# Human-Augment-Analytics/vectordb-retrieval

Hardware: AMD Instinct MI355X
Metric: QPS @ recall@10 (SIFT1M-shaped, 10k-query batch, k=10) (higher is better)
Workload: dtype i8 MFMA scan (i32 accumulate) + exact integer / f64 refine

## Files before the change

### vectordb-retrieval_amd/csrc/refine.hpp

```cpp
#pragma once
#include "common.hpp"
#include "topk.hpp"

namespace vdb {

struct Sq8Rows {
    const unsigned char *codes = nullptr;
    const int32_t *list = nullptr;
    const float *cent = nullptr;
    const float *vmin = nullptr;
    const float *vdiff = nullptr;
};

__device__ __forceinline__ float sq8_decode(unsigned code, float c, float vmin, float vdiff) {
    return c + (vmin + (((float)code + 0.5f) / 255.0f) * vdiff);
}

struct PqRows {
    const unsigned char *codes = nullptr;
    const float *cb = nullptr;
    int M = 0, dsub = 0;
};

struct IvfPqRows {
    const int32_t *list = nullptr;
    const float *cent = nullptr;
    PqRows pq{};
};

struct RefineCommon {
    const float *X;
    const float *Q;
    int64_t N;
    int64_t id_base;
    int D4;
    int metric;
    int k;
    const int64_t *idmap;
    const signed char *X8 = nullptr;
    const int *rowstat = nullptr;
    const signed char *Q8 = nullptr;
    int x8_pitch = 0, cx = 0, D = 0;
    const QueryBatchInfo *info = nullptr;
    Sq8Rows sq8{};
    PqRows pq{};
    IvfPqRows ivfpq{};
};

typedef int refine_int4 __attribute__((ext_vector_type(4)));

template <int U = 16>
__device__ __forceinline__ uint64_t exact_key(const float *__restrict__ x, const float *__restrict__ q, int D4,
                                              int metric) {
    const float4 *xv = reinterpret_cast<const float4 *>(x);
    const float4 *qv = reinterpret_cast<const float4 *>(q);
    double acc = 0.0;
    if (metric == 0) {
#pragma unroll U
        for (int i = 0; i < D4 / 4; ++i) {
            const float4 a = xv[i];
            const float4 b = qv[i];
            double t;
            t = (double)a.x - (double)b.x; acc = fma(t, t, acc);
            t = (double)a.y - (double)b.y; acc = fma(t, t, acc);
            t = (double)a.z - (double)b.z; acc = fma(t, t, acc);
            t = (double)a.w - (double)b.w; acc = fma(t, t, acc);
        }
        return sortable_u64(acc);
    } else {
#pragma unroll U
        for (int i = 0; i < D4 / 4; ++i) {
            const float4 a = xv[i];
            const float4 b = qv[i];
            acc = fma((double)b.x, (double)a.x, acc);
            acc = fma((double)b.y, (double)a.y, acc);
            acc = fma((double)b.z, (double)a.z, acc);
            acc = fma((double)b.w, (double)a.w, acc);
        }
        return sortable_u64(-acc);
    }
}

template <int U = 16>
__device__ __forceinline__ uint64_t exact_key_i8(const signed char *__restrict__ x8, int cx, const float *__restrict__ q,
                                                 int D4, int metric) {
    const int *xw = reinterpret_cast<const int *>(x8);
    const float4 *qv = reinterpret_cast<const float4 *>(q);
    double acc = 0.0;
#pragma unroll U
    for (int i = 0; i < D4 / 4; ++i) {
        const int w = xw[i];
        const float4 b = qv[i];
        const double x0 = (double)((int)(signed char)(w & 0xff) + cx), x1 = (double)((int)(signed char)((w >> 8) & 0xff) + cx);
        const double x2 = (double)((int)(signed char)((w >> 16) & 0xff) + cx), x3 = (double)((w >> 24) + cx);
        if (metric == 0) {
            double t;
            t = x0 - (double)b.x; acc = fma(t, t, acc);
            t = x1 - (double)b.y; acc = fma(t, t, acc);
            t = x2 - (double)b.z; acc = fma(t, t, acc);
            t = x3 - (double)b.w; acc = fma(t, t, acc);
        } else {
            acc = fma((double)b.x, x0, acc);
            acc = fma((double)b.y, x1, acc);
            acc = fma((double)b.z, x2, acc);
            acc = fma((double)b.w, x3, acc);
        }
    }
    return sortable_u64(metric == 0 ? acc : -acc);
}

__device__ __forceinline__ uint64_t sq8_key(const Sq8Rows &s, int64_t row, const float *__restrict__ q, int D4, int metric) {
    const unsigned *cw = reinterpret_cast<const unsigned *>(s.codes + (size_t)row * D4);
    const float4 *cv = reinterpret_cast<const float4 *>(s.cent + (size_t)s.list[row] * D4);
    const float4 *mv = reinterpret_cast<const float4 *>(s.vmin);
    const float4 *dv = reinterpret_cast<const float4 *>(s.vdiff);
    const float4 *qv = reinterpret_cast<const float4 *>(q);
    double acc = 0.0;
#pragma unroll 4
    for (int i = 0; i < D4 / 4; ++i) {
        const unsigned w = cw[i];
        const float4 c = cv[i], m = mv[i], d = dv[i], b = qv[i];
        const double x0 = (double)sq8_decode(w & 0xffu, c.x, m.x, d.x);
        const double x1 = (double)sq8_decode((w >> 8) & 0xffu, c.y, m.y, d.y);
        const double x2 = (double)sq8_decode((w >> 16) & 0xffu, c.z, m.z, d.z);
        const double x3 = (double)sq8_decode(w >> 24, c.w, m.w, d.w);
        if (metric == 0) {
            double t;
            t = x0 - (double)b.x; acc = fma(t, t, acc);
            t = x1 - (double)b.y; acc = fma(t, t, acc);
            t = x2 - (double)b.z; acc = fma(t, t, acc);
            t = x3 - (double)b.w; acc = fma(t, t, acc);
        } else {
            acc = fma((double)b.x, x0, acc);
            acc = fma((double)b.y, x1, acc);
            acc = fma((double)b.z, x2, acc);
            acc = fma((double)b.w, x3, acc);
        }
    }
    return sortable_u64(metric == 0 ? acc : -acc);
}

template <bool RESIDUAL>
__device__ __forceinline__ uint64_t pq_key_body(const PqRows &p, const int32_t *__restrict__ list, const float *__restrict__ cent,
                                                int64_t row, const float *__restrict__ q, int D4, int metric) {
    const unsigned char *cr = p.codes + (size_t)row * p.M;
    const float *cl = RESIDUAL ? cent + (size_t)list[row] * D4 : nullptr;
    double acc = 0.0;
    int d = 0;
    for (int m = 0; m < p.M; ++m) {
        const float *cv = p.cb + ((size_t)m * 256 + cr[m]) * p.dsub;
        for (int j = 0; j < p.dsub; ++j, ++d) {
            const double x = RESIDUAL ? (double)(cl[d] + cv[j]) : (double)cv[j];
            if (metric == 0) {
                const double t = x - (double)q[d];
                acc = fma(t, t, acc);
            } else {
                acc = fma((double)q[d], x, acc);
            }
        }
    }
    for (; d < D4; ++d) {
        if (metric == 0) {
            const double t = 0.0 - (double)q[d];
            acc = fma(t, t, acc);
        } else {
            acc = fma((double)q[d], 0.0, acc);
        }
    }
    return sortable_u64(metric == 0 ? acc : -acc);
}
__device__ __forceinline__ uint64_t pq_key(const PqRows &p, int64_t row, const float *__restrict__ q, int D4, int metric) {
    return pq_key_body<false>(p, nullptr, nullptr, row, q, D4, metric);
}
__device__ __forceinline__ uint64_t ivfpq_key(const IvfPqRows &p, int64_t row, const float *__restrict__ q, int D4, int metric) {
    return pq_key_body<true>(p.pq, p.list, p.cent, row, q, D4, metric);
}

template <int U = 16>
__device__ __forceinline__ uint64_t row_key(const RefineCommon &c, int64_t row, const float *__restrict__ q) {
    if (c.X) return exact_key<U>(c.X + (size_t)row * c.D4, q, c.D4, c.metric);
    if (c.sq8.codes) return sq8_key(c.sq8, row, q, c.D4, c.metric);
    if (c.pq.codes) return pq_key(c.pq, row, q, c.D4, c.metric);
    if (c.ivfpq.pq.codes) return ivfpq_key(c.ivfpq, row, q, c.D4, c.metric);
    return exact_key_i8<U>(c.X8 + (size_t)row * c.x8_pitch, c.cx, q, c.D4, c.metric);
}

template <int QB>
__device__ __forceinline__ void exact_keys(const float *__restrict__ x, const float *const (&q)[QB], int D4, int metric,
                                           uint64_t (&out)[QB]) {
    const float4 *xv = reinterpret_cast<const float4 *>(x);
    double acc[QB];
#pragma unroll
    for (int j = 0; j < QB; ++j) acc[j] = 0.0;
#pragma unroll 4
    for (int i = 0; i < D4 / 4; ++i) {
        const float4 a = xv[i];
#pragma unroll
        for (int j = 0; j < QB; ++j) {
            const float4 b = reinterpret_cast<const float4 *>(q[j])[i];
            if (metric == 0) {
                double t;
                t = (double)a.x - (double)b.x; acc[j] = fma(t, t, acc[j]);
                t = (double)a.y - (double)b.y; acc[j] = fma(t, t, acc[j]);
                t = (double)a.z - (double)b.z; acc[j] = fma(t, t, acc[j]);
                t = (double)a.w - (double)b.w; acc[j] = fma(t, t, acc[j]);
            } else {
                acc[j] = fma((double)b.x, (double)a.x, acc[j]);
                acc[j] = fma((double)b.y, (double)a.y, acc[j]);
                acc[j] = fma((double)b.z, (double)a.z, acc[j]);
                acc[j] = fma((double)b.w, (double)a.w, acc[j]);
            }
        }
    }
#pragma unroll
    for (int j = 0; j < QB; ++j) out[j] = sortable_u64(metric == 0 ? acc[j] : -acc[j]);
}

template <int KPL, int U = 16>
__device__ __forceinline__ void scan_rows(WaveTopK<KPL> &tk, const RefineCommon &c, const float *qptr, int64_t row0,
                                          int64_t row1) {
    const int lane = threadIdx.x & 63;
    if (row1 > c.N) row1 = c.N;
    for (int64_t base = row0; base < row1; base += 64) {
        const int64_t row = base + lane;
        const bool valid = row < row1;
        uint64_t key = ~0ull;
        if (valid) key = row_key<U>(c, row, qptr);
        tk.offer(key, c.idmap ? (valid ? c.idmap[row] : -1) : c.id_base + row, valid);
    }
}

template <int KPL>
__device__ __forceinline__ void write_topk(const WaveTopK<KPL> &tk, int metric, float *D, int64_t *I, double *pk,
                                           int64_t *pi) {
    const int lane = threadIdx.x & 63;
#pragma unroll
    for (int e = 0; e < KPL; ++e) {
        const int s = e * 64 + lane;
        if (s < tk.k) {
            const bool have = s < tk.n;
            const double kv = have ? unsortable_f64(tk.key[e]) : __builtin_inf();
            if (D) {
                float d;
                if (have)
                    d = (float)(metric == 0 ? kv : -kv);
                else
                    d = (metric == 0) ? 3.402823466e+38f : -3.402823466e+38f;
                D[s] = d;
                I[s] = have ? tk.id[e] : -1;
            } else {
                pk[s] = kv;
                pi[s] = have ? tk.id[e] : -1;
            }
        }
    }
}

struct RefineListArgs {
    RefineCommon c;
    int64_t nq;
    const int32_t *cand_rows;
    const int32_t *rescan_rows;
    const int32_t *counts;
    const int32_t *fallback;
    int cand_cap;
    int rescan_cap;
    float *D;
    int64_t *I;
    double *pkeys;
    int64_t *pids;
    int group_shift = -1;
    int f16_shift = 2;
};

template <int KPL, int W>
__device__ __forceinline__ void refine_list_dot8(const RefineListArgs &a, int64_t q, int ncand, int nres, int gshift,
                                                 WaveTopK<KPL> &tk) {
    const int lane = threadIdx.x & 63;
    const RefineCommon &c = a.c;
    const int mode = c.info->i8_mode;
    const int cq = (mode & 3) == 1 ? 127 : -1;
    int qb[W];
    const int *q8 = reinterpret_cast<const int *>(c.Q8 + (size_t)q * c.x8_pitch);
#pragma unroll
    for (int w = 0; w < W; ++w) qb[w] = __builtin_amdgcn_readfirstlane(q8[w]);
    int sq = 0, sqq = 0;
    const float *qf = c.Q + (size_t)q * c.D4;
    for (int d = lane; d < c.D4; d += 64) {
        const int v = (int)qf[d];
        sq += v;
        sqq += v * v;
    }
#pragma unroll
    for (int o = 32; o > 0; o >>= 1) {
        sq += __shfl_xor(sq, o);
        sqq += __shfl_xor(sqq, o);
    }
    const long long cxq = (long long)c.cx * sq - (long long)c.D * c.cx * cq;
    auto key_of = [&](int64_t row) -> uint64_t {
        const refine_int4 *xr = reinterpret_cast<const refine_int4 *>(c.X8 + (size_t)row * c.x8_pitch);
        const int2 st = reinterpret_cast<const int2 *>(c.rowstat)[row];
        int dot = 0;
#pragma unroll
        for (int i = 0; i < W / 4; ++i) {
            const refine_int4 w = xr[i];
            dot = __builtin_amdgcn_sdot4(w.x, qb[4 * i], dot, false);
            dot = __builtin_amdgcn_sdot4(w.y, qb[4 * i + 1], dot, false);
            dot = __builtin_amdgcn_sdot4(w.z, qb[4 * i + 2], dot, false);
            dot = __builtin_amdgcn_sdot4(w.w, qb[4 * i + 3], dot, false);
        }
        const long long xq = -(long long)dot + (long long)cq * st.y + cxq;
        return c.metric == 0 ? sortable_u64((double)((long long)st.x - 2 * xq + sqq)) : sortable_u64(-(double)xq);
    };
    const int32_t *cr = a.cand_rows + (size_t)q * a.cand_cap;
    for (int base = 0; base < (ncand << gshift); base += 64) {
        const int i = base + lane;
        bool valid = i < (ncand << gshift);
        const int64_t row = valid ? (int64_t)cr[i >> gshift] + (i & ((1 << gshift) - 1)) : 0;
        valid = valid && row < c.N;
        const uint64_t key = valid ? key_of(row) : ~0ull;
        tk.offer(key, c.idmap ? (valid ? c.idmap[row] : -1) : c.id_base + row, valid);
    }
    const int32_t *rr = a.rescan_rows + (size_t)q * a.rescan_cap * 2;
    for (int r = 0; r < nres; ++r) {
        const int64_t row0 = rr[2 * r];
        int64_t row1 = rr[2 * r + 1];
        if (row1 > c.N) row1 = c.N;
        for (int64_t base = row0; base < row1; base += 64) {
            const int64_t row = base + lane;
            const bool valid = row < row1;
            const uint64_t key = valid ? key_of(row) : ~0ull;
            tk.offer(key, c.idmap ? (valid ? c.idmap[row] : -1) : c.id_base + row, valid);
        }
    }
}

template <int KPL>
__device__ __forceinline__ void refine_list_body(const RefineListArgs &a, unsigned block) {
    const int lane = threadIdx.x & 63;
    const int64_t q = __builtin_amdgcn_readfirstlane((int)(block * 4 + (threadIdx.x >> 6)));
    if (q >= a.nq) return;
    if (a.fallback[q]) return;
    const float *qptr = a.c.Q + (size_t)q * a.c.D4;
    WaveTopK<KPL> tk;
    tk.init(a.c.k);
    int ncand = a.counts[2 * q];
    int nres = a.counts[2 * q + 1];
    ncand = ncand < a.cand_cap ? ncand : a.cand_cap;
    nres = nres < a.rescan_cap ? nres : a.rescan_cap;
    const int32_t *cr = a.cand_rows + (size_t)q * a.cand_cap;
    const int mode = a.c.info != nullptr ? a.c.info->i8_mode : 0;
    const int gshift = a.group_shift >= 0 ? a.group_shift : mode ? ((mode & 4) ? 3 : 2) : a.f16_shift;
    if (mode != 0 && a.c.X8 != nullptr) {
        if (a.c.x8_pitch == 64) refine_list_dot8<KPL, 16>(a, q, ncand, nres, gshift, tk);
        else refine_list_dot8<KPL, 32>(a, q, ncand, nres, gshift, tk);
    } else {
        for (int base = 0; base < (ncand << gshift); base += 64) {
            const int i = base + lane;
            bool valid = i < (ncand << gshift);
            int64_t row = valid ? (int64_t)cr[i >> gshift] + (i & ((1 << gshift) - 1)) : 0;
            valid = valid && row < a.c.N;
            uint64_t key = ~0ull;
            if (valid) key = row_key(a.c, row, qptr);
            tk.offer(key, a.c.idmap ? (valid ? a.c.idmap[row] : -1) : a.c.id_base + row, valid);
        }
        const int32_t *rr = a.rescan_rows + (size_t)q * a.rescan_cap * 2;
        for (int r = 0; r < nres; ++r) scan_rows<KPL>(tk, a.c, qptr, rr[2 * r], rr[2 * r + 1]);
    }
    const size_t o = (size_t)q * a.c.k;
    write_topk<KPL>(tk, a.c.metric, a.D ? a.D + o : nullptr, a.I ? a.I + o : nullptr, a.pkeys ? a.pkeys + o : nullptr,
                    a.pids ? a.pids + o : nullptr);
}

struct RefineFallbackArgs {
    RefineCommon c;
    const int32_t *fb_list;
    const int32_t *fb_count;
    int max_split;
    int64_t cap_units;
    double *pkeys;
    int64_t *pids;
    int32_t *done;
    float *D;
    int64_t *I;
    double *okeys;
    int64_t *oids;
};

template <int KPL>
__device__ __forceinline__ void refine_fallback_body(const RefineFallbackArgs &a, unsigned block, unsigned nblocks) {
    const int64_t count = *a.fb_count;
    if (count <= 0) return;
    const int lane = threadIdx.x & 63;
    const int64_t waves = (int64_t)nblocks * 4;
    const int64_t wave0 = __builtin_amdgcn_readfirstlane((int)(block * 4 + (threadIdx.x >> 6)));
    int64_t S = waves / count;
    if (S > a.max_split) S = a.max_split;
    if (S > a.cap_units / count) S = a.cap_units / count;
    if (S < 1) S = 1;
    const int64_t rows_per_split = ((a.c.N + S - 1) / S + 63) / 64 * 64;
    for (int64_t u = wave0; u < count * S; u += waves) {
        const int64_t f = u / S;
        const int split = (int)(u - f * S);
        const int64_t q = a.fb_list[f];
        WaveTopK<KPL> tk;
        tk.init(a.c.k);
        scan_rows<KPL, 4>(tk, a.c, a.c.Q + (size_t)q * a.c.D4, (int64_t)split * rows_per_split, (int64_t)(split + 1) * rows_per_split);
        const size_t oq = (size_t)q * a.c.k;
        if (S == 1) {
            if (a.D) write_topk<KPL>(tk, a.c.metric, a.D + oq, a.I + oq, nullptr, nullptr);
            else write_topk<KPL>(tk, a.c.metric, nullptr, nullptr, a.okeys + oq, a.oids + oq);
            continue;
        }
        write_topk<KPL>(tk, a.c.metric, nullptr, nullptr, a.pkeys + (size_t)u * a.c.k, a.pids + (size_t)u * a.c.k);
        __threadfence();
        int last = 0;
        if (lane == 0) last = atomicAdd(&a.done[f], 1) == (int)S - 1;
        last = __builtin_amdgcn_readfirstlane(last);
        if (!last) continue;
        __threadfence();
        if (lane == 0) a.done[f] = 0;
        tk.init(a.c.k);
        const int total = (int)S * a.c.k;
        const size_t o0 = (size_t)f * S * a.c.k;
        for (int base = 0; base < total; base += 64) {
            const int i = base + lane;
            bool valid = i < total;
            uint64_t key = ~0ull;
            int64_t id = -1;
            if (valid) {
                id = __builtin_nontemporal_load(a.pids + o0 + i);
                key = sortable_u64(__builtin_nontemporal_load(a.pkeys + o0 + i));
                valid = id >= 0;
            }
            tk.offer(key, id, valid);
        }
        if (a.D) write_topk<KPL>(tk, a.c.metric, a.D + oq, a.I + oq, nullptr, nullptr);
        else write_topk<KPL>(tk, a.c.metric, nullptr, nullptr, a.okeys + oq, a.oids + oq);
    }
}

template <int KPL>
__global__ __launch_bounds__(256, (KPL == 1 ? 6 : KPL == 2 ? 5 : 1)) void refine_tail_kernel(RefineListArgs la, RefineFallbackArgs fa, unsigned fb_blocks) {
    if (blockIdx.x < fb_blocks) refine_fallback_body<KPL>(fa, blockIdx.x, fb_blocks);
    else refine_list_body<KPL>(la, blockIdx.x - fb_blocks);
}

struct RerankArgs {
    RefineCommon c;
    int64_t nq;
    const int64_t *cand;
    int ncand;
    float *D;
    int64_t *I;
    double *pkeys = nullptr;
    int64_t *pids = nullptr;
    const int64_t *segs = nullptr;
    int nseg = 0;
};

template <int KPL>
__global__ __launch_bounds__(256) void rerank_kernel(RerankArgs a) {
    const int lane = threadIdx.x & 63;
    const int64_t q = __builtin_amdgcn_readfirstlane((int)(blockIdx.x * 4 + (threadIdx.x >> 6)));
    if (q >= a.nq) return;
    const float *qptr = a.c.Q + (size_t)q * a.c.D4;
    WaveTopK<KPL> tk;
    tk.init(a.c.k);
    const int64_t *cr = a.cand + (size_t)q * a.ncand;
    for (int base = 0; base < a.ncand; base += 64) {
        const int i = base + lane;
        bool valid = i < a.ncand;
        const int64_t id = valid ? cr[i] : -1;
        int64_t row = id - a.c.id_base;
        if (a.segs) {
            row = -1;
            for (int j = 0; j < a.nseg; ++j) {
                const int64_t id0 = a.segs[3 * j];
                if (id >= id0 && id < id0 + a.segs[3 * j + 2]) row = a.segs[3 * j + 1] + (id - id0);
            }
        }
        valid = valid && id >= 0 && row >= 0 && row < a.c.N;
        uint64_t key = ~0ull;
        if (valid) key = row_key(a.c, row, qptr);
        tk.offer(key, id, valid);
    }
    const size_t o = (size_t)q * a.c.k;
    write_topk<KPL>(tk, a.c.metric, a.D ? a.D + o : nullptr, a.I ? a.I + o : nullptr, a.pkeys ? a.pkeys + o : nullptr,
                    a.pids ? a.pids + o : nullptr);
}

struct RefineFullArgs {
    RefineCommon c;
    const int32_t *qlist;
    const int32_t *count_ptr;
    int64_t count;
    int S;
    int64_t rows_per_split;
    float *D;
    int64_t *I;
    double *pkeys;
    int64_t *pids;
};

template <int KPL>
__global__ __launch_bounds__(256) void refine_full_kernel(RefineFullArgs a) {
    const int64_t waves_total = (int64_t)gridDim.x * 4;
    const int64_t wave0 = __builtin_amdgcn_readfirstlane((int)(blockIdx.x * 4 + (threadIdx.x >> 6)));
    const int64_t count = a.count_ptr ? (int64_t)*a.count_ptr : a.count;
    const int64_t units = count * a.S;
    for (int64_t u = wave0; u < units; u += waves_total) {
        const int64_t slot = u / a.S;
        const int split = (int)(u - slot * a.S);
        const int64_t q = a.qlist ? (int64_t)a.qlist[slot] : slot;
        const float *qptr = a.c.Q + (size_t)q * a.c.D4;
        WaveTopK<KPL> tk;
        tk.init(a.c.k);
        const int64_t r0 = (int64_t)split * a.rows_per_split;
        scan_rows<KPL>(tk, a.c, qptr, r0, r0 + a.rows_per_split);
        if (a.D) {
            const size_t o = (size_t)q * a.c.k;
            write_topk<KPL>(tk, a.c.metric, a.D + o, a.I + o, nullptr, nullptr);
        } else {
            const size_t o = (size_t)u * a.c.k;
            write_topk<KPL>(tk, a.c.metric, nullptr, nullptr, a.pkeys + o, a.pids + o);
        }
    }
}

template <int KPL, int QB, bool PQ = false>
__global__ __launch_bounds__(256) void refine_full_blocked_kernel(RefineFullArgs a) {
    const int lane = threadIdx.x & 63;
    const int64_t waves_total = (int64_t)gridDim.x * 4;
    const int64_t wave0 = __builtin_amdgcn_readfirstlane((int)(blockIdx.x * 4 + (threadIdx.x >> 6)));
    const int64_t count = a.count_ptr ? (int64_t)*a.count_ptr : a.count;
    const int64_t groups = (count + QB - 1) / QB;
    const int64_t units = groups * a.S;
    for (int64_t u = wave0; u < units; u += waves_total) {
        const int64_t grp = u / a.S;
        const int split = (int)(u - grp * a.S);
        int64_t slot[QB], q[QB];
        const float *qptr[QB];
        WaveTopK<KPL> tk[QB];
#pragma unroll
        for (int j = 0; j < QB; ++j) {
            slot[j] = grp * QB + j;
            const int64_t sj = slot[j] < count ? slot[j] : count - 1;
            q[j] = a.qlist ? (int64_t)a.qlist[sj] : sj;
            qptr[j] = a.c.Q + (size_t)q[j] * a.c.D4;
            tk[j].init(a.c.k);
        }
        const int64_t r0 = (int64_t)split * a.rows_per_split;
        int64_t r1 = r0 + a.rows_per_split;
        if (r1 > a.c.N) r1 = a.c.N;
        for (int64_t base = r0; base < r1; base += 64) {
            const int64_t row = base + lane;
            const bool valid = row < r1;
            uint64_t key[QB];
#pragma unroll
            for (int j = 0; j < QB; ++j) key[j] = ~0ull;
            if (valid) {
                if (PQ) {
#pragma unroll
                    for (int j = 0; j < QB; ++j) key[j] = pq_key(a.c.pq, row, qptr[j], a.c.D4, a.c.metric);
                } else if (a.c.X) {
                    exact_keys<QB>(a.c.X + (size_t)row * a.c.D4, qptr, a.c.D4, a.c.metric, key);
                } else {
#pragma unroll
                    for (int j = 0; j < QB; ++j)
                        key[j] = exact_key_i8<4>(a.c.X8 + (size_t)row * a.c.x8_pitch, a.c.cx, qptr[j], a.c.D4, a.c.metric);
                }
            }
            const int64_t id = a.c.idmap ? (valid ? a.c.idmap[row] : -1) : a.c.id_base + row;
#pragma unroll
            for (int j = 0; j < QB; ++j) tk[j].offer(key[j], id, valid);
        }
#pragma unroll
        for (int j = 0; j < QB; ++j) {
            if (slot[j] < count) {
                if (a.D) {
                    const size_t o = (size_t)q[j] * a.c.k;
                    write_topk<KPL>(tk[j], a.c.metric, a.D + o, a.I + o, nullptr, nullptr);
                } else {
                    const size_t o = (size_t)(slot[j] * a.S + split) * a.c.k;
                    write_topk<KPL>(tk[j], a.c.metric, nullptr, nullptr, a.pkeys + o, a.pids + o);
                }
            }
        }
    }
}

struct MergeArgs {
    const double *pkeys;
    const int64_t *pids;
    int64_t part_stride;
    int64_t slot_stride;
    int nparts;
    int k;
    int metric;
    const int32_t *qlist;
    const int32_t *count_ptr;
    int64_t count;
    float *D;
    int64_t *I;
    double *okeys;
    int64_t *oids;
    const int64_t *seg;
};

template <int KPL>
__global__ __launch_bounds__(256) void merge_kernel(MergeArgs a) {
    const int lane = threadIdx.x & 63;
    const int64_t waves_total = (int64_t)gridDim.x * 4;
    const int64_t wave0 = __builtin_amdgcn_readfirstlane((int)(blockIdx.x * 4 + (threadIdx.x >> 6)));
    const int64_t count = a.count_ptr ? (int64_t)*a.count_ptr : a.count;
    const int total = a.nparts * a.k;
    for (int64_t slot = wave0; slot < count; slot += waves_total) {
        WaveTopK<KPL> tk;
        tk.init(a.k);
        for (int base = 0; base < total; base += 64) {
            const int i = base + lane;
            bool valid = i < total;
            uint64_t key = ~0ull;
            int64_t id = -1;
            if (valid) {
                const int p = i / a.k, j = i - p * a.k;
                const size_t o = (size_t)p * a.part_stride + (size_t)slot * a.slot_stride + j;
                id = a.pids[o];
                key = sortable_u64(a.pkeys[o]);
                valid = id >= 0;
                if (valid && a.seg) {
                    const int64_t *pairs = a.seg + a.nparts + 1;
                    int64_t e = a.seg[p];
                    const int64_t e1 = a.seg[p + 1];
                    while (e + 1 < e1 && pairs[2 * (e + 1)] <= id) ++e;
                    id = pairs[2 * e + 1] + (id - pairs[2 * e]);
                }
            }
            tk.offer(key, id, valid);
        }
        const int64_t q = a.qlist ? (int64_t)a.qlist[slot] : slot;
        const size_t o = (size_t)q * a.k;
        if (a.D)
            write_topk<KPL>(tk, a.metric, a.D + o, a.I + o, nullptr, nullptr);
        else
            write_topk<KPL>(tk, a.metric, nullptr, nullptr, a.okeys + o, a.oids + o);
    }
}

}
```

### vectordb-retrieval_amd/csrc/scan.hpp

```cpp
#pragma once
#include "common.hpp"
#include "prep.hpp"

namespace vdb {

typedef float float16v __attribute__((ext_vector_type(16)));

struct ScanArgs {
    const half8 *panels;
    const float *bias;
    const half8 *qpanels;
    const QueryBatchInfo *info;
    float *bin_m1;
    float *bin_m2;
    float *bin_m3;
    float *sb_m1;
    float *sb_m2;
    int32_t *sb_span;
    int64_t nspans;
    int spans_per_chunk;
    int chunk_rem;
    int nchunks;
    int chunk0;
    int nqtiles;
// ... 235 lines not shown
            }
        }
    };
    auto flush_bin = [&](int64_t span, int bt) {
        if (ITEMS) {
            items_push((int)(span - lspan0) * BPS + bt);
            return;
        }
        const size_t o = (size_t)((span * 2 + h) * BPS + bt) * out_pitch + out_col;
#pragma unroll
        for (int cb = 0; cb < 2; ++cb) {
            __builtin_nontemporal_store(m1[cb], a.bin_m1 + o + cb * 32);
            __builtin_nontemporal_store(m2[cb], a.bin_m2 + o + cb * 32);
            M2[cb] = __builtin_fminf(__builtin_amdgcn_fmed3f(M1[cb], M2[cb], m1[cb]), m2[cb]);
            if (m1[cb] < M1[cb]) Ms[cb] = (int)span;
            M1[cb] = __builtin_fminf(M1[cb], m1[cb]);
            m1[cb] = INF;
            m2[cb] = INF;
        }
    };

    stage_issue(0, 0);
    if (ITEMS) {
        const half8 *ra = reinterpret_cast<const half8 *>(a.qrows + (size_t)(qa < 0 ? 0 : qa) * (16 * KSTEPS)) + h;
        const half8 *rb = reinterpret_cast<const half8 *>(a.qrows + (size_t)(qb < 0 ? 0 : qb) * (16 * KSTEPS)) + h;
        half8 zero;
#pragma unroll
        for (int j = 0; j < 8; ++j) zero[j] = (_Float16)0.f;
#pragma unroll
        for (int ks = 0; ks < KSTEPS; ++ks) {
            b0[ks] = qa < 0 ? zero : ra[ks * 2];
            b1[ks] = qb < 0 ? zero : rb[ks * 2];
        }
    }
    stage_bias_store(0);
    __syncthreads();

    bool idle_wave = !ITEMS && a.nq_valid > 0 && q0 >= a.nq_valid;
    if (ITEMS) idle_wave = __ballot(qa >= 0 || qb >= 0) == 0ull;
    if (idle_wave) {
        for (int st = 0; st < nstages; ++st) {
            if (st + 1 < nstages) {
                stage_issue(st + 1, (st & 1) ^ 1);
                stage_bias_store((st & 1) ^ 1);
            }
            __syncthreads();
        }
        return;
    }

    half8 fr[KSTEPS];
    float16v cin, acc0, acc1;
    if (!late) {
        for (int st = 0; st < nstages; ++st) {
            const int buf = st & 1;
            if (st + 1 < nstages) stage_issue(st + 1, buf ^ 1);
            const half8 *A = lds_a(buf);
            const float4 *B4 = reinterpret_cast<const float4 *>(lds_b(buf)) + h * 4;
            const int ts0 = (st % SPS) * ST;
            read_phase<KSTEPS>(A, B4, fr, cin, lane);
#pragma unroll
            for (int t = 0; t < ST; ++t) {
                __builtin_amdgcn_sched_barrier(0);
                mfma_phase<KSTEPS>(fr, b0, b1, cin, acc0, acc1);
                __builtin_amdgcn_sched_barrier(0);
                if (t + 1 < ST) read_phase<KSTEPS>(A + (t + 1) * KSTEPS * 64, B4 + (t + 1) * 8, fr, cin, lane);
                select_phase<ITEMS, G8>(acc0, acc1, m1, m2, idmask, NEG_INF, (unsigned)(((ts0 + t) % BT) << 2), m3);
            }
            __builtin_amdgcn_sched_barrier(0);
            if (((ts0 + ST) % BT) == 0) flush_bin(span0 + st / SPS, (ts0 + ST) / BT - 1);
            if (st + 1 < nstages) stage_bias_store(buf ^ 1);
            __syncthreads();
        }
    } else {
#pragma unroll
        for (int r = 0; r < 16; ++r) acc0[r] = 3.0e38f;
        acc1 = acc0;
        for (int st = 0; st < nstages; ++st) {
            const int buf = st & 1;
            if (st + 1 < nstages) stage_issue(st + 1, buf ^ 1);
            const half8 *A = lds_a(buf);
            const float4 *B4 = reinterpret_cast<const float4 *>(lds_b(buf)) + h * 4;
            const int ts0 = (st % SPS) * ST;
#pragma unroll
            for (int t = 0; t < ST; ++t) {
                __builtin_amdgcn_sched_barrier(0);
                read_phase<KSTEPS>(A + t * KSTEPS * 64, B4 + t * 8, fr, cin, lane);
                const int tp = (ts0 + t + TPS - 1) % TPS;
                select_phase<ITEMS, G8>(acc0, acc1, m1, m2, idmask, NEG_INF, (unsigned)((tp % BT) << 2), m3);
                if (t == 0 && st > 0 && (ts0 % BT) == 0)
                    flush_bin(span0 + (st * ST - 1) / TPS, tp / BT);
                __builtin_amdgcn_sched_barrier(0);
                mfma_phase<KSTEPS>(fr, b0, b1, cin, acc0, acc1);
            }
            __builtin_amdgcn_sched_barrier(0);
            if (st + 1 < nstages) stage_bias_store(buf ^ 1);
            __syncthreads();
        }
        select_phase<ITEMS, G8>(acc0, acc1, m1, m2, idmask, NEG_INF, (unsigned)((BT - 1) << 2), m3);
        flush_bin(span1 - 1, BPS - 1);
    }
    if (ITEMS)
        for (int r = (int)(span1 - lspan0) * BPS; r & 3; ++r) items_push(r);
    if (ITEMS) return;

    const size_t so = (size_t)(chunk * 2 + h) * a.Qpad + q0 + (lane & 31);
#pragma unroll
    for (int cb = 0; cb < 2; ++cb) {
        a.sb_m1[so + cb * 32] = M1[cb];
        a.sb_m2[so + cb * 32] = M2[cb];
        a.sb_span[so + cb * 32] = Ms[cb];
    }
}

struct SelectArgs {
    const float *bin_m1, *bin_m2, *sb_m1, *sb_m2;
    const int32_t *sb_span;
    const float *eps;
    const QueryBatchInfo *info;
    int64_t nq, Qpad, nspans, N;
    int spans_per_chunk, chunk_rem, nchunks, k;
    int groups;
    int direct_rows;
    int cand_cap, rescan_cap;
    int f16_gmode;
    int32_t *cand_rows;
    int32_t *rescan_rows;
    int32_t *counts;
    int32_t *fallback;
    int32_t *fb_list;
    int32_t *fb_count;
    unsigned long long *stat_counters;
};

__device__ __forceinline__ float select_threshold(float tau, float eps, int i8_mode) {
    return i8_mode ? __int_as_float((__float_as_int(tau) | 63) + __float_as_int(eps)) : tau + 2.0f * eps;
}

template <int VPL>
__global__ __launch_bounds__(256) void select_kernel(SelectArgs a) {
    const int lane = threadIdx.x & 63;
    const int64_t q = __builtin_amdgcn_readfirstlane((int)(blockIdx.x * 4 + (threadIdx.x >> 6)));
    if (q >= a.nq) return;
    const int dbps = a.direct_rows ? kBinRows / a.direct_rows : 0;
    const int nsb = a.direct_rows ? (int)a.nspans * a.groups * dbps : a.nchunks * a.groups;
    unsigned v[VPL];
    float sv[VPL];
#pragma unroll
    for (int e = 0; e < VPL; ++e) sv[e] = a.sb_m1[(size_t)min(e * 64 + lane, nsb - 1) * a.Qpad + q];
#pragma unroll
    for (int e = 0; e < VPL; ++e) asm volatile("" : "+v"(sv[e]));
#pragma unroll
    for (int e = 0; e < VPL; ++e) v[e] = (e * 64 + lane < nsb) ? sortable_u32(sv[e]) : 0xFFFFFFFFu;
    unsigned ans = 0;
    if (VPL >= 4 && a.k <= 64) {
        unsigned lo0 = 0xFFFFFFFFu, lo1 = 0xFFFFFFFFu;
#pragma unroll
        for (int e = 0; e < VPL; ++e) {
            const unsigned x = v[e];
            lo1 = min(lo1, max(lo0, x));
            lo0 = min(lo0, x);
        }
        for (int bit = 31; bit >= 0; --bit) {
            const unsigned trial = ans | ((1u << bit) - 1u);
            const int cnt = __popcll(__ballot(lo0 <= trial)) + __popcll(__ballot(lo1 <= trial));
            if (cnt < a.k) ans |= (1u << bit);
        }
    } else {
        for (int bit = 31; bit >= 0; --bit) {
            const unsigned trial = ans | ((1u << bit) - 1u);
            int cnt = 0;
#pragma unroll
            for (int e = 0; e < VPL; ++e) cnt += __popcll(__ballot(v[e] <= trial));
            if (cnt < a.k) ans |= (1u << bit);
        }
    }
    const float tau = unsortable_f32(ans);
    const int i8_mode = a.info->i8_mode;
    const float that = select_threshold(tau, a.eps[q], i8_mode);
    const int gmode = i8_mode ? i8_mode : a.f16_gmode;
    const bool force_fb = a.info->force_fallback || !(that < 0.9e38f) || nsb < a.k;

    int ncand = 0, nres = 0;
    int32_t *cr = a.cand_rows + (size_t)q * a.cand_cap;
    int32_t *rr = a.rescan_rows + (size_t)q * a.rescan_cap * 2;
    const unsigned long long lt_mask = (1ull << lane) - 1ull;

    if (!force_fb) {
        float sm2v[VPL];
        int spanv[VPL];
#pragma unroll
        for (int e = 0; e < VPL; ++e) sm2v[e] = a.sb_m2[(size_t)min(e * 64 + lane, nsb - 1) * a.Qpad + q];
#pragma unroll
        for (int e = 0; e < VPL; ++e) spanv[e] = a.direct_rows ? 0 : a.sb_span[(size_t)min(e * 64 + lane, nsb - 1) * a.Qpad + q];
#pragma unroll
        for (int e = 0; e < VPL; ++e) asm volatile("" : "+v"(sm2v[e]), "+v"(spanv[e]));
#pragma unroll
        for (int e = 0; e < VPL; ++e) {
            const int s = e * 64 + lane;
            const bool in = s < nsb;
            const float m1 = in ? unsortable_f32(v[e]) : __builtin_inff();
            const bool active = in && (m1 <= that);
            const float sm2 = active ? sm2v[e] : __builtin_inff();
            const int sspan = active ? spanv[e] : 0;
            if (a.direct_rows) {
                const int row0 = (s / dbps) * kBinRows + (s % dbps) * a.direct_rows;
                const bool single = active && !(sm2 <= that), deep = active && !single;
                const unsigned long long smask = __ballot(single), rmask = __ballot(deep);
                if (single) {
                    const int pos = ncand + __popcll(smask & lt_mask);
                    if (pos < a.cand_cap) cr[pos] = row0 + cand_row_offset(__float_as_uint(m1), gmode);
                }
                if (deep) {
                    const int pos = nres + __popcll(rmask & lt_mask);
                    if (pos < a.rescan_cap) {
                        rr[2 * pos] = row0;
                        rr[2 * pos + 1] = row0 + a.direct_rows;
                    }
                }
                ncand += __popcll(smask);
                nres += __popcll(rmask);
                continue;
            }
            const bool single = active && !(sm2 <= that);
            const unsigned long long smask = __ballot(single);
            if (single) {
                const int pos = ncand + __popcll(smask & lt_mask);
                const int hh = s % a.groups;
                const int row = (sspan * a.groups + hh) * kBinRows + cand_row_offset(__float_as_uint(m1), gmode);
                if (pos < a.cand_cap) cr[pos] = row;
            }
            ncand += __popcll(smask);
            unsigned long long dmask = __ballot(active && !single);
            while (dmask) {
                const int src = __ffsll(dmask) - 1;
                dmask &= dmask - 1;
                const int sb = e * 64 + src;
                const int chunk = sb / a.groups, hh = sb % a.groups;
                const int64_t sp0 = chunk_span0(chunk, a.spans_per_chunk, a.chunk_rem);
                int64_t sp1 = chunk_span0(chunk + 1, a.spans_per_chunk, a.chunk_rem);
                if (sp1 > a.nspans) sp1 = a.nspans;
                for (int64_t base = sp0; base < sp1; base += 64) {
                    const int64_t sp = base + lane;
                    bool act = false, resc = false;
                    float bm1 = 0.f;
                    if (sp < sp1) {
                        const size_t o = (size_t)(sp * a.groups + hh) * a.Qpad + q;
                        bm1 = a.bin_m1[o];
                        if (bm1 <= that) {
                            act = true;
                            resc = a.bin_m2[o] <= that;
                        }
                    }
                    const bool cand = act && !resc;
                    const unsigned long long cm = __ballot(cand), rm = __ballot(resc);
                    if (cand) {
                        const int pos = ncand + __popcll(cm & lt_mask);
                        if (pos < a.cand_cap)
                            cr[pos] = (int)((sp * a.groups + hh) * kBinRows + cand_row_offset(__float_as_uint(bm1), gmode));
                    }
                    if (resc) {
                        const int pos = nres + __popcll(rm & lt_mask);
                        if (pos < a.rescan_cap) {
                            rr[2 * pos] = (int)((sp * a.groups + hh) * kBinRows);
                            rr[2 * pos + 1] = rr[2 * pos] + kBinRows;
                        }
                    }
                    ncand += __popcll(cm);
                    nres += __popcll(rm);
                }
            }
        }
    }
    const bool fb = force_fb || ncand > a.cand_cap || nres > a.rescan_cap;
    if (lane == 0) {
        a.counts[2 * q] = fb ? 0 : ncand;
        a.counts[2 * q + 1] = fb ? 0 : nres;
        a.fallback[q] = fb ? 1 : 0;
        if (fb) {
            const int pos = atomicAdd(a.fb_count, 1);
            a.fb_list[pos] = (int)q;
            stat_add(a.stat_counters, q, 2, 1ull);
        } else {
            stat_add(a.stat_counters, q, 0, (unsigned long long)ncand);
            stat_add(a.stat_counters, q, 1, (unsigned long long)nres);
        }
    }
}

template <int V, int LPQ>
__global__ __launch_bounds__(256, 1) void select_kernel_v2(SelectArgs a) {
    constexpr int QPW = 64 / LPQ;
    constexpr int kDeepCap = 48;
    __shared__ int s_cnt[4][QPW][3];
    __shared__ int s_deep[4][QPW][kDeepCap];
    const int lane = threadIdx.x & 63, wave = threadIdx.x >> 6;
    const int qi = lane / LPQ, part = lane % LPQ;
    const int64_t q = ((int64_t)blockIdx.x * 4 + wave) * QPW + qi;
    const bool qvalid = q < a.nq;
    const int nsb = a.nchunks * a.groups;
    if (part < 3) s_cnt[wave][qi][part] = 0;
    unsigned v[V];
    float sv[V];
#pragma unroll
    for (int e = 0; e < V; ++e) sv[e] = a.sb_m1[(size_t)min(e * LPQ + part, nsb - 1) * a.Qpad + q];
#pragma unroll
    for (int e = 0; e < V; ++e) asm volatile("" : "+v"(sv[e]));
#pragma unroll
    for (int e = 0; e < V; ++e) v[e] = (e * LPQ + part < nsb) ? sortable_u32(sv[e]) : 0xFFFFFFFFu;
    unsigned ans = 0;
    for (int bit = 31; bit >= 0; --bit) {
        const unsigned trial = ans | ((1u << bit) - 1u);
        int cnt = 0;
#pragma unroll
        for (int e = 0; e < V; ++e) cnt += (v[e] <= trial) ? 1 : 0;
#pragma unroll
        for (int o = 1; o < LPQ; o <<= 1) cnt += __shfl_xor(cnt, o);
        if (cnt < a.k) ans |= (1u << bit);
    }
    const float tau = unsortable_f32(ans);
    const int i8_mode = a.info->i8_mode;
    const float that = select_threshold(tau, qvalid ? a.eps[q] : 0.f, i8_mode);
    const int gmode = i8_mode ? i8_mode : a.f16_gmode;
    const bool force_fb = a.info->force_fallback || !(that < 0.9e38f) || nsb < a.k;
    __syncthreads();
    int *cnt_c = &s_cnt[wave][qi][0], *cnt_r = &s_cnt[wave][qi][1], *cnt_d = &s_cnt[wave][qi][2];
    int *deep = &s_deep[wave][qi][0];
    bool deep_overflow = false;
    if (qvalid && !force_fb) {
        int32_t *cr = a.cand_rows + (size_t)q * a.cand_cap;
        float sm2v[V];
        int spanv[V];
#pragma unroll
        for (int e = 0; e < V; ++e) {
            const int s = e * LPQ + part;
            const bool act = (s < nsb) && (unsortable_f32(v[e]) <= that);
            sm2v[e] = act ? a.sb_m2[(size_t)s * a.Qpad + q] : __builtin_inff();
            spanv[e] = act ? a.sb_span[(size_t)s * a.Qpad + q] : 0;
        }
#pragma unroll
        for (int e = 0; e < V; ++e) {
            const int s = e * LPQ + part;
            if (s >= nsb) continue;
            const float m1 = unsortable_f32(v[e]);
            if (!(m1 <= that)) continue;
            const int hh = s % a.groups;
            if (!(sm2v[e] <= that)) {
                const int pos = atomicAdd(cnt_c, 1);
                if (pos < a.cand_cap)
                    cr[pos] = (spanv[e] * a.groups + hh) * kBinRows + cand_row_offset(__float_as_uint(m1), gmode);
            } else {
                const int pos = atomicAdd(cnt_d, 1);
                if (pos < kDeepCap) deep[pos] = s;
            }
        }
    }
    __syncthreads();
    {
        const int nd_q = (qvalid && !force_fb) ? *cnt_d : 0;
        int nd_max = nd_q;
#pragma unroll
        for (int o = 1; o < 64; o <<= 1) nd_max = max(nd_max, __shfl_xor(nd_max, o));
        if (nd_q > kDeepCap) deep_overflow = true;
        int32_t *cr = a.cand_rows + (size_t)q * a.cand_cap;
        int32_t *rr = a.rescan_rows + (size_t)q * a.rescan_cap * 2;
        for (int d = 0; d < nd_max && d < kDeepCap; ++d) {
            if (d >= nd_q) continue;
            const int s = deep[d];
            const int chunk = s / a.groups, hh = s % a.groups;
            const int64_t sp0 = chunk_span0(chunk, a.spans_per_chunk, a.chunk_rem);
            int64_t sp1 = chunk_span0(chunk + 1, a.spans_per_chunk, a.chunk_rem);
            if (sp1 > a.nspans) sp1 = a.nspans;
            for (int64_t sp = sp0 + part; sp < sp1; sp += LPQ) {
                const size_t o = (size_t)(sp * a.groups + hh) * a.Qpad + q;
                const float bm1 = a.bin_m1[o];
                if (!(bm1 <= that)) continue;
                if (a.bin_m2[o] <= that) {
                    const int pos = atomicAdd(cnt_r, 1);
                    if (pos < a.rescan_cap) {
                        rr[2 * pos] = (int)((sp * a.groups + hh) * kBinRows);
                        rr[2 * pos + 1] = rr[2 * pos] + kBinRows;
                    }
                } else {
                    const int pos = atomicAdd(cnt_c, 1);
                    if (pos < a.cand_cap)
                        cr[pos] = (int)((sp * a.groups + hh) * kBinRows + cand_row_offset(__float_as_uint(bm1), gmode));
                }
            }
        }
    }
    __syncthreads();
    if (qvalid && part == 0) {
        const int ncand = *cnt_c, nres = *cnt_r;
        const bool fb = force_fb || deep_overflow || ncand > a.cand_cap || nres > a.rescan_cap;
        a.counts[2 * q] = fb ? 0 : ncand;
        a.counts[2 * q + 1] = fb ? 0 : nres;
        a.fallback[q] = fb ? 1 : 0;
        if (fb) {
            const int pos = atomicAdd(a.fb_count, 1);
            a.fb_list[pos] = (int)q;
            stat_add(a.stat_counters, q, 2, 1ull);
        } else {
            stat_add(a.stat_counters, q, 0, (unsigned long long)ncand);
            stat_add(a.stat_counters, q, 1, (unsigned long long)nres);
        }
    }
}

}
```

Measured before the change: 11.82 million.

## Batch header and list loads in refine and deep-select for latency hiding

The refine kernel now issues all per-query header loads (fallback flag, counts, mode, first candidate window, query int8 words and the first floats) together before any dependency, then broadcasts them with readlane. Candidate and rescan list entries are fetched one wave-wide window at a time and shuffled, instead of being loaded per step. In select_kernel_v2, the info and eps loads are hoisted early, and deep-bin probing handles four deep slots at once so their bin loads are in flight together. This targets exposed memory latency from serialized scalar loads, at the cost of more registers and more compiler-barrier complexity.

```diff
diff --git a/vectordb-retrieval_amd/csrc/refine.hpp b/vectordb-retrieval_amd/csrc/refine.hpp
--- a/vectordb-retrieval_amd/csrc/refine.hpp
+++ b/vectordb-retrieval_amd/csrc/refine.hpp
@@ -273,23 +273,43 @@
     int f16_shift = 2;
 };
 
+struct RefineListHeader {
+    int32_t cw;
+    int rw_touch;
+    int q8w;
+    float qv0, qv1;
+};
+
+__device__ __forceinline__ int32_t list_entry(const int32_t *__restrict__ list, int cap, int i, int &win, int32_t &w) {
+    const int lane = threadIdx.x & 63;
+    const int need = __builtin_amdgcn_readfirstlane(i >> 6);
+    if (need != win) {
+        win = need;
+        w = list[min(need * 64 + lane, cap - 1)];
+    }
+    return __shfl(w, i & 63);
+}
+
 template <int KPL, int W>
-__device__ __forceinline__ void refine_list_dot8(const RefineListArgs &a, int64_t q, int ncand, int nres, int gshift,
-                                                 WaveTopK<KPL> &tk) {
+__device__ __forceinline__ void refine_list_dot8(const RefineListArgs &a, int64_t q, int ncand, int nres, int gshift, int mode,
+                                                 RefineListHeader &hd, WaveTopK<KPL> &tk) {
     const int lane = threadIdx.x & 63;
     const RefineCommon &c = a.c;
-    const int mode = c.info->i8_mode;
     const int cq = (mode & 3) == 1 ? 127 : -1;
     int qb[W];
-    const int *q8 = reinterpret_cast<const int *>(c.Q8 + (size_t)q * c.x8_pitch);
-#pragma unroll
-    for (int w = 0; w < W; ++w) qb[w] = __builtin_amdgcn_readfirstlane(q8[w]);
+#pragma unroll
+    for (int w = 0; w < W; ++w) qb[w] = __builtin_amdgcn_readlane(hd.q8w, w);
     int sq = 0, sqq = 0;
-    const float *qf = c.Q + (size_t)q * c.D4;
-    for (int d = lane; d < c.D4; d += 64) {
-        const int v = (int)qf[d];
-        sq += v;
-        sqq += v * v;
+    {
+        const int v0 = lane < c.D4 ? (int)hd.qv0 : 0, v1 = 64 + lane < c.D4 ? (int)hd.qv1 : 0;
+        sq = v0 + v1;
+        sqq = v0 * v0 + v1 * v1;
+        const float *qf = c.Q + (size_t)q * c.D4;
+        for (int d = 128 + lane; d < c.D4; d += 64) {
+            const int v = (int)qf[d];
+            sq += v;
+            sqq += v * v;
+        }
     }
 #pragma unroll
     for (int o = 32; o > 0; o >>= 1) {
@@ -297,13 +317,19 @@
         sqq += __shfl_xor(sqq, o);
     }
     const long long cxq = (long long)c.cx * sq - (long long)c.D * c.cx * cq;
-    auto key_of = [&](int64_t row) -> uint64_t {
+    refine_int4 xw[W / 4];
+    int2 st;
+    auto request = [&](int row) {
         const refine_int4 *xr = reinterpret_cast<const refine_int4 *>(c.X8 + (size_t)row * c.x8_pitch);
-        const int2 st = reinterpret_cast<const int2 *>(c.rowstat)[row];
+#pragma unroll
+        for (int i = 0; i < W / 4; ++i) xw[i] = xr[i];
+        st = reinterpret_cast<const int2 *>(c.rowstat)[row];
+    };
+    auto key_now = [&]() -> uint64_t {
         int dot = 0;
 #pragma unroll
         for (int i = 0; i < W / 4; ++i) {
-            const refine_int4 w = xr[i];
+            const refine_int4 w = xw[i];
             dot = __builtin_amdgcn_sdot4(w.x, qb[4 * i], dot, false);
             dot = __builtin_amdgcn_sdot4(w.y, qb[4 * i + 1], dot, false);
             dot = __builtin_amdgcn_sdot4(w.z, qb[4 * i + 2], dot, false);
@@ -312,26 +338,40 @@
         const long long xq = -(long long)dot + (long long)cq * st.y + cxq;
         return c.metric == 0 ? sortable_u64((double)((long long)st.x - 2 * xq + sqq)) : sortable_u64(-(double)xq);
     };
+    auto run = [&](int nsteps, auto row_of) {
+        for (int t = 0; t < nsteps; ++t) {
+            bool valid;
+            const int row = row_of(t, valid);
+            uint64_t key = ~0ull;
+            if (valid) {
+                request(row);
+                key = key_now();
+            }
+            tk.offer(key, c.idmap ? (valid ? c.idmap[row] : -1) : c.id_base + row, valid);
+        }
+    };
     const int32_t *cr = a.cand_rows + (size_t)q * a.cand_cap;
-    for (int base = 0; base < (ncand << gshift); base += 64) {
-        const int i = base + lane;
-        bool valid = i < (ncand << gshift);
-        const int64_t row = valid ? (int64_t)cr[i >> gshift] + (i & ((1 << gshift) - 1)) : 0;
-        valid = valid && row < c.N;
-        const uint64_t key = valid ? key_of(row) : ~0ull;
-        tk.offer(key, c.idmap ? (valid ? c.idmap[row] : -1) : c.id_base + row, valid);
-    }
+    const int nrows = ncand << gshift;
+    int cwin = 0;
+    run((nrows + 63) >> 6, [&](int t, bool &valid) -> int {
+        const int i = t * 64 + lane;
+        const int32_t e = list_entry(cr, a.cand_cap, i >> gshift, cwin, hd.cw);
+        const int64_t row = (int64_t)e + (i & ((1 << gshift) - 1));
+        valid = i < nrows && row < c.N;
+        return (int)row;
+    });
     const int32_t *rr = a.rescan_rows + (size_t)q * a.rescan_cap * 2;
+    int2 rw{};
     for (int r = 0; r < nres; ++r) {
-        const int64_t row0 = rr[2 * r];
-        int64_t row1 = rr[2 * r + 1];
+        if ((r & 63) == 0) rw = reinterpret_cast<const int2 *>(rr)[min(r + lane, a.rescan_cap - 1)];
+        const int64_t row0 = __builtin_amdgcn_readlane(rw.x, r & 63);
+        int64_t row1 = __builtin_amdgcn_readlane(rw.y, r & 63);
         if (row1 > c.N) row1 = c.N;
-        for (int64_t base = row0; base < row1; base += 64) {
-            const int64_t row = base + lane;
-            const bool valid = row < row1;
-            const uint64_t key = valid ? key_of(row) : ~0ull;
-            tk.offer(key, c.idmap ? (valid ? c.idmap[row] : -1) : c.id_base + row, valid);
-        }
+        run((int)((row1 - row0 + 63) >> 6), [&](int t, bool &valid) -> int {
+            const int64_t row = row0 + (int64_t)t * 64 + lane;
+            valid = row < row1;
+            return (int)row;
+        });
     }
 }
 
@@ -340,32 +380,58 @@
     const int lane = threadIdx.x & 63;
     const int64_t q = __builtin_amdgcn_readfirstlane((int)(block * 4 + (threadIdx.x >> 6)));
     if (q >= a.nq) return;
-    if (a.fallback[q]) return;
     const float *qptr = a.c.Q + (size_t)q * a.c.D4;
+    const int32_t *cr = a.cand_rows + (size_t)q * a.cand_cap;
+    const int32_t *rr = a.rescan_rows + (size_t)q * a.rescan_cap * 2;
+    const bool rows8 = a.c.X8 != nullptr && a.c.Q8 != nullptr;
+    int zl = 0;
+    asm volatile("" : "+v"(zl));
+    RefineListHeader hd;
+    int fbv = a.fallback[q + zl];
+    int ncv = a.counts[2 * q + zl];
+    int nrv = a.counts[2 * q + 1 + zl];
+    int mdv = 0;
+    if (a.c.info != nullptr) mdv = (&a.c.info->i8_mode)[zl];
+    hd.cw = cr[min(lane, a.cand_cap - 1)];
+    hd.rw_touch = rr[2 * min(lane, a.rescan_cap - 1)];
+    hd.qv0 = hd.qv1 = 0.f;
+    hd.q8w = 0;
+    if (rows8) {
+        hd.q8w = reinterpret_cast<const int *>(a.c.Q8 + (size_t)q * a.c.x8_pitch)[min(lane, a.c.x8_pitch / 4 - 1)];
+        hd.qv0 = qptr[min(lane, a.c.D4 - 1)];
+        hd.qv1 = qptr[min(64 + lane, a.c.D4 - 1)];
+    }
+    __builtin_amdgcn_sched_barrier(0);
+    asm volatile("" : "+v"(fbv), "+v"(ncv), "+v"(nrv), "+v"(mdv));
+    asm volatile("" : "+v"(hd.cw), "+v"(hd.rw_touch), "+v"(hd.q8w), "+v"(hd.qv0), "+v"(hd.qv1));
+    const int fbq = __builtin_amdgcn_readfirstlane(fbv), mode = __builtin_amdgcn_readfirstlane(mdv);
+    int ncand = __builtin_amdgcn_readfirstlane(ncv), nres = __builtin_amdgcn_readfirstlane(nrv);
+    if (fbq) return;
     WaveTopK<KPL> tk;
     tk.init(a.c.k);
-    int ncand = a.counts[2 * q];
-    int nres = a.counts[2 * q + 1];
     ncand = ncand < a.cand_cap ? ncand : a.cand_cap;
     nres = nres < a.rescan_cap ? nres : a.rescan_cap;
-    const int32_t *cr = a.cand_rows + (size_t)q * a.cand_cap;
-    const int mode = a.c.info != nullptr ? a.c.info->i8_mode : 0;
     const int gshift = a.group_shift >= 0 ? a.group_shift : mode ? ((mode & 4) ? 3 : 2) : a.f16_shift;
-    if (mode != 0 && a.c.X8 != nullptr) {
-        if (a.c.x8_pitch == 64) refine_list_dot8<KPL, 16>(a, q, ncand, nres, gshift, tk);
-        else refine_list_dot8<KPL, 32>(a, q, ncand, nres, gshift, tk);
+    if (mode != 0 && rows8) {
+        if (a.c.x8_pitch == 64) refine_list_dot8<KPL, 16>(a, q, ncand, nres, gshift, mode, hd, tk);
+        else refine_list_dot8<KPL, 32>(a, q, ncand, nres, gshift, mode, hd, tk);
     } else {
+        int cwin = 0;
         for (int base = 0; base < (ncand << gshift); base += 64) {
             const int i = base + lane;
             bool valid = i < (ncand << gshift);
-            int64_t row = valid ? (int64_t)cr[i >> gshift] + (i & ((1 << gshift) - 1)) : 0;
+            const int32_t e = list_entry(cr, a.cand_cap, i >> gshift, cwin, hd.cw);
+            int64_t row = valid ? (int64_t)e + (i & ((1 << gshift) - 1)) : 0;
             valid = valid && row < a.c.N;
             uint64_t key = ~0ull;
             if (valid) key = row_key(a.c, row, qptr);
             tk.offer(key, a.c.idmap ? (valid ? a.c.idmap[row] : -1) : a.c.id_base + row, valid);
         }
-        const int32_t *rr = a.rescan_rows + (size_t)q * a.rescan_cap * 2;
-        for (int r = 0; r < nres; ++r) scan_rows<KPL>(tk, a.c, qptr, rr[2 * r], rr[2 * r + 1]);
+        int2 rw{};
+        for (int r = 0; r < nres; ++r) {
+            if ((r & 63) == 0) rw = reinterpret_cast<const int2 *>(rr)[min(r + lane, a.rescan_cap - 1)];
+            scan_rows<KPL>(tk, a.c, qptr, __builtin_amdgcn_readlane(rw.x, r & 63), __builtin_amdgcn_readlane(rw.y, r & 63));
+        }
     }
     const size_t o = (size_t)q * a.c.k;
     write_topk<KPL>(tk, a.c.metric, a.D ? a.D + o : nullptr, a.I ? a.I + o : nullptr, a.pkeys ? a.pkeys + o : nullptr,
diff --git a/vectordb-retrieval_amd/csrc/scan.hpp b/vectordb-retrieval_amd/csrc/scan.hpp
--- a/vectordb-retrieval_amd/csrc/scan.hpp
+++ b/vectordb-retrieval_amd/csrc/scan.hpp
@@ -561,8 +561,12 @@
     if (part < 3) s_cnt[wave][qi][part] = 0;
     unsigned v[V];
     float sv[V];
+    const int i8_mode = a.info->i8_mode;
+    const int info_ffb = a.info->force_fallback;
+    float epsq = a.eps[qvalid ? q : a.nq - 1];
 #pragma unroll
     for (int e = 0; e < V; ++e) sv[e] = a.sb_m1[(size_t)min(e * LPQ + part, nsb - 1) * a.Qpad + q];
+    __builtin_amdgcn_sched_barrier(0);
 #pragma unroll
     for (int e = 0; e < V; ++e) asm volatile("" : "+v"(sv[e]));
 #pragma unroll
@@ -578,10 +582,10 @@
         if (cnt < a.k) ans |= (1u << bit);
     }
     const float tau = unsortable_f32(ans);
-    const int i8_mode = a.info->i8_mode;
-    const float that = select_threshold(tau, qvalid ? a.eps[q] : 0.f, i8_mode);
+    asm volatile("" : "+v"(epsq));
+    const float that = select_threshold(tau, qvalid ? epsq : 0.f, i8_mode);
     const int gmode = i8_mode ? i8_mode : a.f16_gmode;
-    const bool force_fb = a.info->force_fallback || !(that < 0.9e38f) || nsb < a.k;
+    const bool force_fb = info_ffb || !(that < 0.9e38f) || nsb < a.k;
     __syncthreads();
     int *cnt_c = &s_cnt[wave][qi][0], *cnt_r = &s_cnt[wave][qi][1], *cnt_d = &s_cnt[wave][qi][2];
     int *deep = &s_deep[wave][qi][0];
@@ -616,34 +620,57 @@
     }
     __syncthreads();
     {
-        const int nd_q = (qvalid && !force_fb) ? *cnt_d : 0;
+        constexpr int kDeepWidth = 4;
+        const int nd_q = (qvalid && !force_fb) ? min(*cnt_d, kDeepCap) : 0;
         int nd_max = nd_q;
 #pragma unroll
         for (int o = 1; o < 64; o <<= 1) nd_max = max(nd_max, __shfl_xor(nd_max, o));
-        if (nd_q > kDeepCap) deep_overflow = true;
+        if (qvalid && !force_fb && *cnt_d > kDeepCap) deep_overflow = true;
         int32_t *cr = a.cand_rows + (size_t)q * a.cand_cap;
         int32_t *rr = a.rescan_rows + (size_t)q * a.rescan_cap * 2;
-        for (int d = 0; d < nd_max && d < kDeepCap; ++d) {
-            if (d >= nd_q) continue;
-            const int s = deep[d];
-            const int chunk = s / a.groups, hh = s % a.groups;
-            const int64_t sp0 = chunk_span0(chunk, a.spans_per_chunk, a.chunk_rem);
-            int64_t sp1 = chunk_span0(chunk + 1, a.spans_per_chunk, a.chunk_rem);
-            if (sp1 > a.nspans) sp1 = a.nspans;
-            for (int64_t sp = sp0 + part; sp < sp1; sp += LPQ) {
-                const size_t o = (size_t)(sp * a.groups + hh) * a.Qpad + q;
-                const float bm1 = a.bin_m1[o];
-                if (!(bm1 <= that)) continue;
-                if (a.bin_m2[o] <= that) {
-                    const int pos = atomicAdd(cnt_r, 1);
-                    if (pos < a.rescan_cap) {
-                        rr[2 * pos] = (int)((sp * a.groups + hh) * kBinRows);
-                        rr[2 * pos + 1] = rr[2 * pos] + kBinRows;
-                    }
-                } else {
-                    const int pos = atomicAdd(cnt_c, 1);
-                    if (pos < a.cand_cap)
-                        cr[pos] = (int)((sp * a.groups + hh) * kBinRows + cand_row_offset(__float_as_uint(bm1), gmode));
+        auto decide = [&](int64_t sp, int hh, float bm1, float bm2) {
+            if (!(bm1 <= that)) return;
+            if (bm2 <= that) {
+                const int pos = atomicAdd(cnt_r, 1);
+                if (pos < a.rescan_cap) {
+                    rr[2 * pos] = (int)((sp * a.groups + hh) * kBinRows);
+                    rr[2 * pos + 1] = rr[2 * pos] + kBinRows;
+                }
+            } else {
+                const int pos = atomicAdd(cnt_c, 1);
+                if (pos < a.cand_cap)
+                    cr[pos] = (int)((sp * a.groups + hh) * kBinRows + cand_row_offset(__float_as_uint(bm1), gmode));
+            }
+        };
+        for (int d0 = 0; d0 < nd_max; d0 += kDeepWidth) {
+            int hh[kDeepWidth];
+            int64_t sp[kDeepWidth], sp1[kDeepWidth];
+            float bm1[kDeepWidth], bm2[kDeepWidth];
+#pragma unroll
+            for (int j = 0; j < kDeepWidth; ++j) {
+                const bool have = d0 + j < nd_q;
+                const int s = have ? deep[d0 + j] : 0;
+                const int chunk = s / a.groups;
+                hh[j] = s % a.groups;
+                sp[j] = chunk_span0(chunk, a.spans_per_chunk, a.chunk_rem) + part;
+                sp1[j] = chunk_span0(chunk + 1, a.spans_per_chunk, a.chunk_rem);
+                if (sp1[j] > a.nspans) sp1[j] = a.nspans;
+                if (!have) sp1[j] = 0;
+                const size_t o = sp[j] < sp1[j] ? (size_t)(sp[j] * a.groups + hh[j]) * a.Qpad + q : (size_t)q;
+                bm1[j] = a.bin_m1[o];
+                bm2[j] = a.bin_m2[o];
+            }
+            __builtin_amdgcn_sched_barrier(0);
+#pragma unroll
+            for (int j = 0; j < kDeepWidth; ++j) asm volatile("" : "+v"(bm1[j]), "+v"(bm2[j]));
+#pragma unroll
+            for (int j = 0; j < kDeepWidth; ++j) {
+                if (sp[j] < sp1[j]) decide(sp[j], hh[j], bm1[j], bm2[j]);
+                for (int64_t s2 = sp[j] + LPQ; s2 < sp1[j]; s2 += LPQ) {
+                    const size_t o = (size_t)(s2 * a.groups + hh[j]) * a.Qpad + q;
+                    float c1 = a.bin_m1[o], c2 = a.bin_m2[o];
+                    asm volatile("" : "+v"(c1), "+v"(c2));
+                    decide(s2, hh[j], c1, c2);
                 }
             }
         }
```

Result: no change. 11.88 million, median of 6 (+0.5%).
